# VinAIResearch/Point-Unet

Hardware: AMD Instinct MI355X
Metric: points_per_sec_forward (higher is better)
Workload: dtype f32

## Files before the change

point-unet_amd/csrc/attpool.h:

```cpp
#pragma once

#include "common.h"
#include "rowgemm.h"

namespace ps {

struct Att32Weights {
    const float* w1 = nullptr;
    const float* w2 = nullptr;
    const float* wb1 = nullptr;
    const float* wb2 = nullptr;
    const float* w1b = nullptr;
    const float* w2b = nullptr;
    const float* wb1b = nullptr;
    const float* wb2b = nullptr;
};
void pack_b3(const float* W, int cin, int cout, uint16_t* out);
void pack_b3_locse(const float* W1, int cout, uint16_t* out);
void pack_p32(const float* W, int cin, int cout, float* out);
void pack_p32_locse(const float* W1, int cout, float* out);

struct AttStage {
    const float* xyz = nullptr;
    const int32_t* idx = nullptr;
    const int32_t* order = nullptr;
    const float* fg = nullptr;
    const PackedLinear* lfa1 = nullptr;
    const PackedLinear* lfa2 = nullptr;
    const PackedLinear* wbot = nullptr;
    const PackedLinear* wfull = nullptr;
    int ldf = 0;
    float* agg = nullptr;
    int64_t n_total = 0, n_cloud = 0;
    int d = 0, k = 16;
    const Att32Weights* p32 = nullptr;
};

bool att_pool32_fits(const AttStage& s);
int att_pool32_stage(ps_context* c, const AttStage& s);
bool att_pool32b_fits(const AttStage& s);
int att_pool32b_stage(ps_context* c, const AttStage& s);

int att_pool_stage(ps_context* c, const AttStage& s);
int att_pool16_stage(ps_context* c, const AttStage& s);

}
```

point-unet_amd/csrc/attpool.hip:

```cpp
#include "attpool.h"
#include "mfma_tile.h"

namespace ps {

struct AttArgs {
    const float* xyz;
    const int32_t* idx;
    const int32_t* order;
    const float* fg;
    const float* w1p; const float* b1;
    const float* w2p; const float* b2;
    const float* wbp;
    const float* wfp;
    float* agg;
    int n_total, n_cloud, ldf;
};

struct PointWalk {
    int t, end, stride;
    __device__ __forceinline__ PointWalk(int n_total, int units_per_wg, int unit_in_wg)
    {
        const int per_xcd = (n_total + 7) >> 3;
        const int xcd = blockIdx.x & 7, slot = blockIdx.x >> 3, slots = gridDim.x >> 3;
        t = xcd * per_xcd + slot * units_per_wg + unit_in_wg;
// ... 436 lines not shown
static int dispatch_direct(ps_context* c, int d, const AttArgs& a)
{
    switch (d) {
        case 16: return launch_att_direct<16, STAGE, KN>(c, a);
        case 32: return launch_att_direct<32, STAGE, KN>(c, a);
        default: set_error("att_pool(direct): d_out %d is not a compiled size (16, 32: the weights live in registers)", d); return PS_EINVAL;
    }
}

template <int D, int STAGE, int KN>
static int launch_att(ps_context* c, const AttArgs& a)
{
    constexpr int H = D / 2, PITCH = H + 2;
    constexpr size_t per_wave = (size_t)KN * PITCH * (STAGE == 2 ? 2 : 1) * sizeof(float);
    if (D >= 256 && a.n_total < 16384) {
        constexpr int WAVES = 4;
        const size_t smem = per_wave;
        auto kern = att_kernel<D, STAGE, KN, WAVES, true>;
        if (smem > 48 * 1024) PS_HIP(hipFuncSetAttribute(reinterpret_cast<const void*>(kern), hipFuncAttributeMaxDynamicSharedMemorySize, (int)smem));
        const int blocks = (std::min(a.n_total, 256 * 16) + 7) & ~7;
        hipLaunchKernelGGL(kern, dim3(blocks), dim3(WAVES * 64), smem, c->stream, a);
        PS_HIP(hipGetLastError());
        return PS_OK;
    }
    constexpr int WAVES = per_wave * 4 <= 160 * 1024 ? 4 : (per_wave * 2 <= 160 * 1024 ? 2 : 1);
    static_assert(per_wave * WAVES <= 160 * 1024, "attention tile does not fit the LDS");
    const size_t smem = per_wave * WAVES;
    auto kern = att_kernel<D, STAGE, KN, WAVES, false>;
    if (smem > 48 * 1024) PS_HIP(hipFuncSetAttribute(reinterpret_cast<const void*>(kern), hipFuncAttributeMaxDynamicSharedMemorySize, (int)smem));
    const int blocks = (std::min(ceil_div(a.n_total, WAVES), 256 * 8) + 7) & ~7;
    hipLaunchKernelGGL(kern, dim3(blocks), dim3(WAVES * 64), smem, c->stream, a);
    PS_HIP(hipGetLastError());
    return PS_OK;
}

template <int STAGE, int KN>
static int dispatch_d(ps_context* c, int d, const AttArgs& a)
{
    switch (d) {
        case 16: return launch_att<16, STAGE, KN>(c, a);
        case 32: return launch_att<32, STAGE, KN>(c, a);
        case 64: return launch_att<64, STAGE, KN>(c, a);
        case 128: return launch_att<128, STAGE, KN>(c, a);
        case 256: return launch_att<256, STAGE, KN>(c, a);
        case 512: return launch_att<512, STAGE, KN>(c, a);
        default: set_error("att_pool: d_out %d is not a compiled size (16,32,64,128,256,512)", d); return PS_EINVAL;
    }
}

int att_pool_stage(ps_context* c, const AttStage& s)
{
    if (c->att_bf16x3 && att_pool32b_fits(s)) return att_pool32b_stage(c, s);
    if (att_pool32_fits(s)) return att_pool32_stage(c, s);
    return att_pool16_stage(c, s);
}

int att_pool16_stage(ps_context* c, const AttStage& s)
{
    AttArgs a;
    a.xyz = s.xyz; a.idx = s.idx; a.order = s.order; a.fg = s.fg;
    a.w1p = s.lfa1->wp; a.b1 = s.lfa1->bias;
    a.w2p = s.lfa2 ? s.lfa2->wp : nullptr; a.b2 = s.lfa2 ? s.lfa2->bias : nullptr;
    a.wbp = s.wbot ? s.wbot->wp : nullptr;
    a.wfp = s.wfull ? s.wfull->wp : nullptr;
    a.agg = s.agg;
    a.n_total = (int)s.n_total; a.n_cloud = (int)s.n_cloud;
    a.ldf = s.ldf;
    if (s.n_total <= 0) return PS_OK;
    const int stage = s.lfa2 ? 2 : 1;
    if (s.wfull) {
        PS_CHECK((uint64_t)s.n_total * (uint64_t)std::max(s.d, std::max(s.ldf, 3 * 1)) < (1ull << 32) && (uint64_t)s.n_total * s.k < (1ull << 32),
                 "att_pool: level too large for 32-bit element offsets");
        if (s.k == 16) return stage == 1 ? dispatch_direct<1, 16>(c, s.d, a) : dispatch_direct<2, 16>(c, s.d, a);
        if (s.k == 32) return stage == 1 ? dispatch_direct<1, 32>(c, s.d, a) : dispatch_direct<2, 32>(c, s.d, a);
        set_error("att_pool: k_n %d is not a compiled size (16, 32)", s.k);
        return PS_EINVAL;
    }
    if (s.k == 16) return stage == 1 ? dispatch_d<1, 16>(c, s.d, a) : dispatch_d<2, 16>(c, s.d, a);
    if (s.k == 32) return stage == 1 ? dispatch_d<1, 32>(c, s.d, a) : dispatch_d<2, 32>(c, s.d, a);
    set_error("att_pool: k_n %d is not a compiled size (16, 32)", s.k);
    return PS_EINVAL;
}

}
```

point-unet_amd/csrc/common.h:

```cpp
#pragma once

#include <hip/hip_runtime.h>

#include <cstdarg>
#include <cstdint>
#include <cstdio>
#include <cstring>
#include <map>
#include <string>
#include <vector>

#include "../../include/pointseg.h"
#include "../../include/pointseg_train_ops.h"

namespace ps {

void set_error(const char* fmt, ...);

#define PS_HIP(expr)                                                                                  \
    do {                                                                                              \
        hipError_t _e = (expr);                                                                       \
        if (_e != hipSuccess) {                                                                       \
            ps::set_error("%s failed: %s (%s:%d)", #expr, hipGetErrorString(_e), __FILE__, __LINE__); \
            return PS_EHIP;                                                                           \
// ... 71 lines not shown
int pack_cache_finish_recording(ps_context* c, PackCache& pc);
int pack_cache_replay(ps_context* c, PackCache& pc);
void pack_cache_clear(PackCache& pc);
int pack_batch_ops(ps_context* c, const PackJob* table, int n);
int pack_batch_b3(ps_context* c, const PackJob* table, int n);
}

namespace ps {
struct Tuning {
    double gemm32b_min_flops = 3e8;
    int gemm32b_rw = 0, gemm32b_cw = 0;
    bool gemm32_no_sk8 = false;
    bool att64_gemm = true;
    int att64_occ = 0;
    bool att_no_split = false;
    int64_t wgrad_b3_min_rows = 0;
    int64_t gemm_b3_min_rows = 0;
    int64_t wgrad_wgs = 512;
    bool bn_slice = false;
    bool inv_bucket = true;
    int inv_tile = 4096;
    bool gather_reduce_ordered = true;
    int maxpool_bwd_ordered = 1;
    bool train_act_bf16 = true;
    int train_att_gemm_split = -1;
    bool train_att_gemm = true;
    bool train_att128_fwd_gemm = true;
    bool train_fuse_residual = true;
    bool train_merge_syncbn = true;
    int convbn_max_c = 64;
    int convbn_rect_max = 1 << 30;
    bool wgrad_debug = false;
};
void tuning_from_env(Tuning& t);
}

struct ps_context {
    int device = 0;
    ps::Tuning tune;
    hipStream_t own_stream = nullptr;
    hipStream_t stream = nullptr;
    ps::Arena knn_arena;
    ps::Arena net_arena;
    ps::Arena sample_arena;
    ps::DevBuf stage_in;
    ps::DevBuf stage_out;
    ps::DevBuf red_ws;
    ps::DevBuf wgrad_ws;
    ps::PackCache* pack_cache = nullptr;
    ps::DevBuf ops_ring[4];
    int ops_ring_pos = 0;
    bool att_bf16x3 = true;
    bool regchain_b3 = true;
    bool train_b3 = true;
    bool conv_w_transposed = false;
    bool att_df_accum = false;
    const int32_t* walk_order = nullptr;
    int64_t walk_order_n = 0;
    bool pool_bwd_overwrite = false;
    bool train_bf16 = false;
    bool train_act_bf16 = false;
    bool mid_lds_attr = false;
    size_t chain_lds_attr = 48 * 1024;
    std::map<const void*, size_t> regchain_lds_attr;
    bool deferred = false;
    int32_t* h_flags = nullptr;
    unsigned pending_mask = 0;
    uint64_t builds = 0;
    uint64_t samples = 0;
    uint64_t volume_samples = 0;
    uint64_t flag_serial[8] = {};
    int flag_kind[8] = {};
    int flag_slot = 0;
    int sticky_rc = 0;
    std::string sticky_msg;
    hipEvent_t flag_ev[8] = {};
    std::vector<char> host_ring[8];
    int ring_pos = 0;
    std::vector<char>& ring_next() { ring_pos = (ring_pos + 1) & 7; return host_ring[ring_pos]; }
    int check_deferred();
    int check_flag_slot(int s);
    int defer_status(const void* d_words, size_t bytes, int kind, uint64_t serial);
    struct PinSlot { void* p = nullptr; size_t cap = 0; hipEvent_t ev = nullptr; bool busy = false; };
    PinSlot pin[16];
    int pin_pos = 0;
    int upload_async(void* dst, const void* src, size_t bytes);
    bool timing = false;
    std::string timing_only;
    std::vector<ps::StageTimer> stages;
    std::vector<hipEvent_t> event_pool;
    size_t event_next = 0;
    int cur_stage = -1;
    hipEvent_t cur_start = nullptr;

    hipEvent_t get_event();
    void stage_begin(const char* name);
    void stage_end(int launches);
};

namespace ps {
struct Stage {
    ps_context* c;
    int n;
    bool on = false;
    Stage(ps_context* ctx, const char* name, int launches = 1) : c(ctx), n(launches)
    {
// ... 49 lines not shown
```

point-unet_amd/csrc/context.hip:

```cpp
#include "common.h"
#include "kdtree_build.h"

#include <cstdlib>

namespace ps {

static thread_local char g_err[512] = "";

void set_error(const char* fmt, ...)
{
    va_list ap;
    va_start(ap, fmt);
    vsnprintf(g_err, sizeof g_err, fmt, ap);
    va_end(ap);
}

int DevBuf::reserve(size_t bytes)
{
    if (bytes <= cap) return PS_OK;
    if (p) {
        hipError_t e = hipDeviceSynchronize();
        if (e != hipSuccess) {
            set_error("hipDeviceSynchronize failed: %s", hipGetErrorString(e));
            return PS_EHIP;
// ... 168 lines not shown
    if (num("PS_GEMM32B_MIN_FLOPS", v) && v >= 0) t.gemm32b_min_flops = v;
    if (num("PS_GEMM32B_RW", v) && (v == 1 || v == 2)) t.gemm32b_rw = (int)v;
    if (num("PS_GEMM32B_CW", v) && (v == 1 || v == 2)) t.gemm32b_cw = (int)v;
    t.gemm32_no_sk8 = std::getenv("PS_GEMM32_NO_SK8") != nullptr;
    flag("PS_ATT64_GEMM", t.att64_gemm);
    if (num("PS_ATT64_OCC", v) && (v == 1 || v == 2)) t.att64_occ = (int)v;
    t.att_no_split = std::getenv("PS_ATT_NO_SPLIT") != nullptr;
    clampi("PS_WGRAD_B3_MIN_ROWS", 0, 1ll << 40, t.wgrad_b3_min_rows);
    clampi("PS_GEMM_B3_MIN_ROWS", 0, 1ll << 40, t.gemm_b3_min_rows);
    clampi("PS_WGRAD_WGS", 64, 4096, t.wgrad_wgs);
    flag("PS_BN_SLICE", t.bn_slice);
    flag("PS_INV_BUCKET", t.inv_bucket);
    if (num("PS_INV_TILE", v) && (v == 4096 || v == 6144 || v == 8192)) t.inv_tile = (int)v;
    flag("PS_GATHER_REDUCE_ORDERED", t.gather_reduce_ordered);
    if (num("PS_MAXPOOL_BWD_ORDERED", v)) t.maxpool_bwd_ordered = v != 0;
    flag("PS_TRAIN_ACT_BF16", t.train_act_bf16);
    if (num("PS_TRAIN_ATT_GEMM_SPLIT", v)) t.train_att_gemm_split = v < 0 ? -1 : (v != 0);
    flag("PS_TRAIN_ATT_GEMM", t.train_att_gemm);
    flag("PS_TRAIN_ATT128_FWD_GEMM", t.train_att128_fwd_gemm);
    flag("PS_TRAIN_FUSE_RESIDUAL", t.train_fuse_residual);
    flag("PS_TRAIN_MERGE_SYNCBN", t.train_merge_syncbn);
    if (num("PS_CONVBN_MAX_C", v) && v >= 0 && v <= 4096) t.convbn_max_c = (int)v;
    if (num("PS_CONVBN_RECT_MAX", v) && v >= 0) t.convbn_rect_max = v > (double)(1 << 30) ? 1 << 30 : (int)v;
    t.wgrad_debug = std::getenv("PS_WGRAD_DEBUG") != nullptr;
#else
    (void)t;
#endif
}
}

extern "C" {
const char* ps_version(void) { return "pointseg-hip 0.1 gfx950"; }
int ps_abi_version(void) { return PS_ABI_VERSION; }

int ps_create(int device, ps_context** out)
{
    PS_CHECK(out != nullptr, "ps_create: out is NULL");
    int count = 0;
    PS_HIP(hipGetDeviceCount(&count));
    PS_CHECK(device >= 0 && device < count, "ps_create: device %d out of range (%d devices)", device, count);
    PS_HIP(hipSetDevice(device));
    ps_context* c = new ps_context();
    c->device = device;
    hipError_t e = hipStreamCreateWithFlags(&c->own_stream, hipStreamNonBlocking);
    if (e != hipSuccess) {
        delete c;
        ps::set_error("hipStreamCreate failed: %s", hipGetErrorString(e));
        return PS_EHIP;
    }
    c->stream = c->own_stream;
    ps::tuning_from_env(c->tune);
#ifdef PS_TUNING_ENV
    if (const char* v = std::getenv("PS_REGCHAIN_B3")) c->regchain_b3 = std::atof(v) != 0;
#endif
    *out = c;
    return PS_OK;
}

int ps_destroy(ps_context* c)
{
    if (!c) return PS_OK;
    (void)hipSetDevice(c->device);
    (void)hipStreamSynchronize(c->stream);
    c->knn_arena.buf.release();
    c->net_arena.buf.release();
    c->sample_arena.buf.release();
    c->stage_in.release();
    c->stage_out.release();
    c->red_ws.release();
    c->wgrad_ws.release();
    for (auto& b : c->ops_ring) b.release();
    if (c->h_flags) (void)hipHostFree(c->h_flags);
    for (auto& e : c->flag_ev)
        if (e) (void)hipEventDestroy(e);
    for (auto& s : c->pin) {
        if (s.p) (void)hipHostFree(s.p);
        if (s.ev) (void)hipEventDestroy(s.ev);
    }
    for (hipEvent_t e : c->event_pool) (void)hipEventDestroy(e);
    if (c->own_stream) (void)hipStreamDestroy(c->own_stream);
    delete c;
    return PS_OK;
}

int ps_set_stream(ps_context* c, void* hip_stream)
{
    PS_CHECK(c != nullptr, "ps_set_stream: ctx is NULL");
    c->stream = static_cast<hipStream_t>(hip_stream);
    return PS_OK;
}

int ps_synchronize(ps_context* c)
{
    PS_CHECK(c != nullptr, "ps_synchronize: ctx is NULL");
    PS_HIP(hipStreamSynchronize(c->stream));
    return c->check_deferred();
}

int ps_set_train_gemm_bf16(ps_context* c, int on)
{
    PS_CHECK(c != nullptr, "ps_set_train_gemm_bf16: ctx is NULL");
    c->train_bf16 = on != 0;
    return PS_OK;
}

int ps_set_train_act_bf16(ps_context* c, int on)
// ... 75 lines not shown
```

point-unet_amd/csrc/debug_hooks.h:

```cpp
#ifndef POINTSEG_DEBUG_H
#define POINTSEG_DEBUG_H
#include "../../include/pointseg.h"
#ifdef __cplusplus
extern "C" {
#endif
int ps_debug_knn_host(const float* support, const float* queries, int64_t B, int64_t n_support,
                      int64_t n_queries, int64_t K, int32_t* out_idx);
int ps_debug_kdtree_host(const float* support, int64_t n, int32_t* vind, int32_t* nodes, float* pts,
                         int32_t* root_depth, float* bbox);
int ps_debug_kdtree_device(ps_context* ctx, const float* support, int64_t n, int32_t* vind, int32_t* nodes,
                           float* pts, int32_t* root_depth, float* bbox);
#define PS_DEBUG_KDTREE_STATS 22
int ps_debug_kdtree_device_set(ps_context* ctx, const float* support, const int32_t* n, int64_t T, const int32_t* want_copy, int32_t* vind,
                               int32_t* nodes, float* pts, int32_t* fat, int32_t* root_depth, float* bbox, float* copy, int32_t* stats);
int ps_debug_pack_weights(const float* W, int cin, int cout, int ntb, float* out);
int ps_debug_pack_b3(const float* W, int cin, int cout, uint16_t* out);
int ps_debug_gemm32(ps_context* ctx, int split_bf16, const float* x1, int ld1, int c1, const int32_t* g1, const float* x2, int ld2, int c2,
                    const int32_t* g2, int gm, int gn, const float* W, const float* bias, int64_t R, int cout, int leaky, float* y, int ldy);
int ps_debug_gemm32_plan(ps_context* ctx, int split_bf16, int64_t R, int cin, int cout, int* out4);

typedef struct ps_debug_chain_layer {
    const float* W;
    const float* bias;
    int cin, cout, leaky;
    float* y;
    int ldy;
    const float* extra;
    int ld_extra, c_extra;
    const int32_t* extra_gather;
} ps_debug_chain_layer;
typedef struct ps_debug_chain_desc {
    int n_layers;
    ps_debug_chain_layer layer[4];
    const float* x1; const int32_t* g1; int ld1, c1, g1m, g1n;
    const float* x2; const int32_t* g2; int ld2, c2, g2m, g2n;
    int64_t R;
} ps_debug_chain_desc;
int ps_debug_chain(ps_context* ctx, const ps_debug_chain_desc* d, int form);
int ps_debug_chain_plan(const ps_debug_chain_desc* d, int* out4);
int ps_debug_set_regchain_b3(ps_context* ctx, int on);
int ps_debug_att_stage(ps_randla* net, int level, int stage, int form, const float* xyz, const int32_t* idx, const int32_t* order, const float* fg,
                       int64_t n_total, int64_t n_cloud, float* agg);

int ps_debug_set_tuning(ps_context* ctx, const char* field, double value);
int ps_debug_get_tuning(ps_context* ctx, const char* field, double* value);
int ps_debug_tuning_fields(char* buf, int cap);
int ps_debug_volume_sample_args_size(void);

int64_t ps_debug_scan_words(int64_t n);
int64_t ps_debug_sort_words(int64_t n);
int ps_debug_scan_launches(int64_t n);
int ps_debug_sort_launches(int64_t n, int bits);
int ps_debug_scan_u32(ps_context* ctx, const uint32_t* in, uint32_t* out, int64_t n, uint32_t* work);
int ps_debug_sort_pairs(ps_context* ctx, int key_bytes, void* k0, void* k1, uint32_t* v0, uint32_t* v1, int64_t n, int bits, uint32_t* work,
                        int* which_out);
int ps_debug_reduce_partials(ps_context* ctx, int form, const void* part, int n_part, int nv, int n0, void* out0, void* out1);

#ifdef __cplusplus
}
#endif
#endif
```

point-unet_amd/csrc/debug_hooks.hip:

```cpp
#include "common.h"

#include <cstring>
#include <vector>
#include "kdtree_build.h"
#include "kdtree_host.h"
#include "rowgemm.h"
#include "attpool.h"
#include "debug_hooks.h"
#include "randla_net.h"
#include "reduce_partials.h"
#include "sortscan.h"

using namespace ps;

extern "C" int ps_debug_volume_sample_args_size(void) { return (int)sizeof(ps_volume_sample_args); }

extern "C" int ps_debug_pack_weights(const float* W, int cin, int cout, int ntb, float* out)
{
    PS_CHECK(W && out && (ntb == 1 || ntb == 2 || ntb == 4), "ps_debug_pack_weights: bad argument");
    pack_weights(W, cin, cout, ntb, out);
    return PS_OK;
}

extern "C" int ps_debug_pack_b3(const float* W, int cin, int cout, uint16_t* out)
// ... 149 lines not shown
    float* dev = nullptr;
    PS_HIP(hipMalloc(reinterpret_cast<void**>(&dev), total * sizeof(float)));
    int rc = PS_OK;
    if (hipMemcpyAsync(dev, host.data(), host.size() * sizeof(float), hipMemcpyHostToDevice, c->stream) != hipSuccess) {
        set_error("ps_debug_chain: upload failed");
        rc = PS_EHIP;
    }
    for (int i = 0; i < b.n; ++i) {
        b.L[i].wp = dev + wp_off[i];
        b.L[i].bias = dev + b_off[i];
        b.L[i].wq = wq_off[i] ? dev + wq_off[i] : nullptr;
    }
    if (rc == PS_OK) {
        if (form == 0) {
            ChainCache cache;
            if (rowchain_fits(b.steps, b.n, b.s1, b.s2)) rc = rowchain(c, b.steps, b.n, b.s1, b.s2, d->R, &cache);
            else { set_error("ps_debug_chain: the chain fits neither chain kernel (channels above %d, mismatched, or a gathered extra)", kChainMaxC); rc = PS_EINVAL; }
            (void)hipStreamSynchronize(c->stream);
            cache.clear();
        } else if (form == 1) {
            if (regchain_fits(b.steps, b.n, b.s1, b.s2)) rc = regchain(c, b.steps, b.n, b.s1, b.s2, d->R, nullptr);
            else { set_error("ps_debug_chain: not one of regchain's compiled chain shapes"); rc = PS_EINVAL; }
        } else if (form == 2) {
            if (rowchain_lds_plan(b.steps, b.n, b.s1, b.s2, d->R).form == 2) rc = rowchain_lds(c, b.steps, b.n, b.s1, b.s2, d->R);
            else { set_error("ps_debug_chain: the chain does not fit the LDS-staged kernel (channels above %d, mismatched, or a gathered extra)", kChainMaxC); rc = PS_EINVAL; }
        } else {
            RowSrc in1 = b.s1, in2 = b.s2;
            for (int i = 0; i < b.n && rc == PS_OK; ++i) {
                const ChainStep& st = b.steps[i];
                if (i > 0) {
                    in2 = RowSrc();
                    if (st.extra.x) in2 = st.extra;
                }
                float* out = st.y ? st.y : dev + tmp_off[i];
                const int ldo = st.y ? st.ldy : b.L[i].cout;
                rc = rowgemm(c, b.L[i], in1, in2, d->R, out, ldo);
                in1 = RowSrc();
                in1.x = out; in1.ld = ldo; in1.c = b.L[i].cout;
            }
        }
    }
    (void)hipStreamSynchronize(c->stream);
    (void)hipFree(dev);
    return rc;
}

extern "C" int ps_debug_set_regchain_b3(ps_context* c, int on)
{
    PS_CHECK(c && (on == 0 || on == 1), "ps_debug_set_regchain_b3: bad argument");
    c->regchain_b3 = on != 0;
    return PS_OK;
}

extern "C" int ps_debug_att_stage(ps_randla* net, int level, int stage, int form, const float* xyz, const int32_t* idx, const int32_t* order,
                                  const float* fg, int64_t n_total, int64_t n_cloud, float* agg)
{
    PS_CHECK(net && xyz && idx && fg && agg, "ps_debug_att_stage: NULL argument");
    PS_CHECK(net->have_weights, "ps_debug_att_stage: weights not set");
    PS_CHECK(level >= 0 && level < net->cfg.num_layers && (stage == 1 || stage == 2) && form >= 0 && form <= 3, "ps_debug_att_stage: bad level / stage / form");
    PS_CHECK(n_total >= 0 && n_cloud >= 1 && n_total % n_cloud == 0, "ps_debug_att_stage: n_total must be a whole number of clouds");
    ps_context* c = net->ctx;
    PS_HIP(hipSetDevice(c->device));
    const EncLevel& e = net->enc[level];
    const int d = e.d, h = d / 2;
    const bool use_g = d >= 64;
    AttStage s;
    s.xyz = xyz; s.idx = idx; s.order = order; s.fg = fg; s.lfa1 = &e.lfa1; s.agg = agg;
    s.n_total = n_total; s.n_cloud = n_cloud; s.d = d; s.k = net->cfg.k_n; s.ldf = use_g ? h + d : h;
    s.p32 = e.has_p32 ? &e.p32 : nullptr;
    s.lfa2 = stage == 2 ? &e.lfa2 : nullptr;
    s.wbot = use_g ? (stage == 1 ? &e.bot1 : &e.bot2) : nullptr;
    s.wfull = use_g ? nullptr : (stage == 1 ? &e.full1 : &e.full2);
    int rc = PS_EINVAL;
    if (form == 0) rc = att_pool_stage(c, s);
    else if (form == 1 && att_pool32b_fits(s)) rc = att_pool32b_stage(c, s);
    else if (form == 2 && att_pool32_fits(s)) rc = att_pool32_stage(c, s);
    else if (form == 3) rc = att_pool16_stage(c, s);
    else set_error("ps_debug_att_stage: the level (d = %d, %lld rows) does not fit the 32x32 form %d", d, (long long)n_total, form);
    (void)hipStreamSynchronize(c->stream);
    return rc;
}

static bool is_bool(double v) { return v == 0 || v == 1; }
static bool is_int_in(double v, double lo, double hi) { return v >= lo && v <= hi && v == (double)(int64_t)v; }

#define PS_TUNING_FIELDS(X)                                                \
    X(gemm32b_min_flops, v >= 0 && v <= 1e300)                             \
    X(gemm32b_rw, v == 0 || v == 1 || v == 2)                              \
    X(gemm32b_cw, v == 0 || v == 1 || v == 2)                              \
    X(gemm32_no_sk8, is_bool(v))                                           \
    X(att64_gemm, is_bool(v))                                              \
    X(att64_occ, v == 0 || v == 1 || v == 2)                               \
    X(att_no_split, is_bool(v))                                            \
    X(wgrad_b3_min_rows, is_int_in(v, 0, (double)(1ll << 40)))             \
    X(gemm_b3_min_rows, is_int_in(v, 0, (double)(1ll << 40)))              \
    X(wgrad_wgs, is_int_in(v, 64, 4096))                                   \
    X(bn_slice, is_bool(v))                                                \
    X(inv_bucket, is_bool(v))                                              \
    X(inv_tile, v == 4096 || v == 6144 || v == 8192)                       \
    X(gather_reduce_ordered, is_bool(v))                                   \
    X(maxpool_bwd_ordered, is_bool(v))                                     \
    X(train_act_bf16, is_bool(v))                                          \
    X(train_att_gemm_split, v == -1 || v == 0 || v == 1)                   \
    X(train_att_gemm, is_bool(v))                                          \
    X(train_att128_fwd_gemm, is_bool(v))                                   \
    X(train_fuse_residual, is_bool(v))                                     \
    X(train_merge_syncbn, is_bool(v))                                      \
    X(convbn_max_c, is_int_in(v, 0, 4096))                                 \
    X(convbn_rect_max, is_int_in(v, 0, (double)(1 << 30)))                 \
    X(wgrad_debug, is_bool(v))

extern "C" int ps_debug_set_tuning(ps_context* c, const char* field, double v)
{
    PS_CHECK(c && field, "ps_debug_set_tuning: NULL argument");
#define PS_SET(f, ok)                                                                                 \
    if (std::strcmp(field, #f) == 0) {                                                                \
        PS_CHECK(ok, "ps_debug_set_tuning: %g is not a value %s is compiled for", v, #f);             \
        c->tune.f = static_cast<decltype(c->tune.f)>(v);                                              \
        return PS_OK;                                                                                 \
    }
    PS_TUNING_FIELDS(PS_SET)
#undef PS_SET
    PS_CHECK(false, "ps_debug_set_tuning: no knob named '%s'", field);
}

extern "C" int ps_debug_get_tuning(ps_context* c, const char* field, double* out)
{
    PS_CHECK(c && field && out, "ps_debug_get_tuning: NULL argument");
#define PS_GET(f, ok)                               \
    if (std::strcmp(field, #f) == 0) {              \
        *out = static_cast<double>(c->tune.f);      \
        return PS_OK;                               \
    }
    PS_TUNING_FIELDS(PS_GET)
// ... 188 lines not shown
```

point-unet_amd/csrc/randla.hip:

```cpp
#include "attpool.h"
#include "common.h"
#include "randla_net.h"
#include "rowgemm.h"

#include <memory>

namespace ps {

template <int KN>
__global__ __launch_bounds__(256) void pool_max_kernel(const float* __restrict__ feat, const int32_t* __restrict__ idx, const int32_t* __restrict__ order,
                                                       float* __restrict__ out, int rows_out, int m_cloud, int n_cloud, int K, int c4 ,
                                                       unsigned char* __restrict__ ties )
{
    const int per_xcd = (rows_out + 7) >> 3;
    const int xcd = blockIdx.x & 7;
    const size_t lim = (size_t)min(rows_out, (xcd + 1) * per_xcd) * c4;
    for (size_t t = (size_t)xcd * per_xcd * c4 + (size_t)(blockIdx.x >> 3) * 256 + threadIdx.x; t < lim; t += (size_t)(gridDim.x >> 3) * 256) {
        const int r = (int)(t / c4), q = (int)(t - (size_t)r * c4);
        const int row = order ? (r / m_cloud) * m_cloud + order[r] : r;
        const int base = (row / m_cloud) * n_cloud;
        const int32_t* ix = idx + (size_t)row * K;
        const float4* f4 = reinterpret_cast<const float4*>(feat);
        float4 m;
        if constexpr (KN > 0) {
// ... 193 lines not shown
        return host.data() + off;
    };
    size_t si = 0;
    auto W = [&](size_t i) { return blob + net->specs[i].w_off; };
    auto Bv = [&](size_t i) { return blob + net->specs[i].b_off; };
    const ps_randla_config& cfg = net->cfg;
    emit(net->fc0, W(si), Bv(si), cfg.in_channels, 8, 1);
    ++si;
    net->enc.assign(cfg.num_layers, EncLevel());
    int d_in = 8;
    std::vector<float> tmp;
    for (int i = 0; i < cfg.num_layers; ++i) {
        EncLevel& e = net->enc[i];
        const int d = cfg.d_out[i], h = d / 2;
        e.d = d; e.d_in = d_in;
        e.has_p32 = d >= 64;
        if (e.has_p32) {
            pack_p32_locse(W(si + 1), h, emit_raw(&e.p32.w1, (size_t)(h / 32) * 5 * 64));
            auto scaled = [&](const float* src, size_t count) {
                tmp.resize(count);
                for (size_t t = 0; t < count; ++t) tmp[t] = (float)((double)src[t] * 1.4426950408889634);
                return tmp.data();
            };
            pack_p32(scaled(W(si + 2) + (size_t)h * d, (size_t)h * d), h, d, emit_raw(&e.p32.wb1, (size_t)h * d));
            pack_p32(W(si + 4), h, h, emit_raw(&e.p32.w2, (size_t)h * h));
            pack_p32(scaled(W(si + 5) + (size_t)h * d, (size_t)h * d), h, d, emit_raw(&e.p32.wb2, (size_t)h * d));
            if (d == 64 || d == 128 || d == 256 || d == 512) {
                pack_b3_locse(W(si + 1), h, reinterpret_cast<uint16_t*>(emit_raw(&e.p32.w1b, (size_t)(h / 32) * 3 * 64 * 4)));
                pack_b3(scaled(W(si + 2) + (size_t)h * d, (size_t)h * d), h, d, reinterpret_cast<uint16_t*>(emit_raw(&e.p32.wb1b, (size_t)h * d * 3 / 2)));
                pack_b3(W(si + 4), h, h, reinterpret_cast<uint16_t*>(emit_raw(&e.p32.w2b, (size_t)h * h * 3 / 2)));
                pack_b3(scaled(W(si + 5) + (size_t)h * d, (size_t)h * d), h, d, reinterpret_cast<uint16_t*>(emit_raw(&e.p32.wb2b, (size_t)h * d * 3 / 2)));
            }
        }
        emit(e.mlp1, W(si), Bv(si), d_in, h, 1); ++si;
        emit(e.lfa1, W(si), Bv(si), 10, h, 1); ++si;
        emit(e.top1, W(si), nullptr, h, d, 0);
        emit(e.bot1, W(si) + (size_t)h * d, nullptr, h, d, 0);
        {
            std::vector<float> sc((size_t)d * d);
            for (size_t t = 0; t < sc.size(); ++t) sc[t] = (float)((double)W(si)[t] * 1.4426950408889634);
            emit(e.full1, sc.data(), nullptr, d, d, 0);
        }
        ++si;
        emit(e.att1mlp, W(si), Bv(si), d, h, 1); ++si;
        emit(e.lfa2, W(si), Bv(si), h, h, 1); ++si;
        emit(e.top2, W(si), nullptr, h, d, 0);
        emit(e.bot2, W(si) + (size_t)h * d, nullptr, h, d, 0);
        {
            std::vector<float> sc((size_t)d * d);
            for (size_t t = 0; t < sc.size(); ++t) sc[t] = (float)((double)W(si)[t] * 1.4426950408889634);
            emit(e.full2, sc.data(), nullptr, d, d, 0);
        }
        ++si;
        emit(e.att2mlp, W(si), Bv(si), d, d, 1); ++si;
        tmp.assign((size_t)(d + d_in) * 2 * d + 2 * d, 0.f);
        std::memcpy(tmp.data(), W(si), sizeof(float) * (size_t)d * 2 * d);
        std::memcpy(tmp.data() + (size_t)d * 2 * d, W(si + 1), sizeof(float) * (size_t)d_in * 2 * d);
        float* bsum = tmp.data() + (size_t)(d + d_in) * 2 * d;
        for (int k = 0; k < 2 * d; ++k) bsum[k] = Bv(si)[k] + Bv(si + 1)[k];
        emit(e.mlp2sc, tmp.data(), bsum, d + d_in, 2 * d, 1);
        si += 2;
        d_in = 2 * d;
    }
    emit(net->decoder0, W(si), Bv(si), d_in, d_in, 1); ++si;
    net->dec.assign(cfg.num_layers, PackedLinear());
    for (int j = 0; j < cfg.num_layers; ++j) {
        emit(net->dec[j], W(si), Bv(si), net->specs[si].cin, net->specs[si].cout, 1);
        ++si;
    }
    emit(net->fc1, W(si), Bv(si), net->specs[si].cin, 64, 1); ++si;
    emit(net->fc2, W(si), Bv(si), 64, 32, 1); ++si;
    emit(net->fc, W(si), Bv(si), 32, cfg.num_classes, 0); ++si;

    PS_TRY(net->wbuf.reserve(host.size() * sizeof(float)));
    PS_HIP(hipMemcpyAsync(net->wbuf.p, host.data(), host.size() * sizeof(float), hipMemcpyHostToDevice, c->stream));
    PS_HIP(hipStreamSynchronize(c->stream));
    for (auto& p : pend) {
        p.L->wp = net->wbuf.as<float>() + p.wp_off;
        p.L->bias = net->wbuf.as<float>() + p.b_off;
        p.L->wq = p.wq_off ? net->wbuf.as<float>() + p.wq_off : nullptr;
        p.L->w32 = p.w32_off ? net->wbuf.as<float>() + p.w32_off : nullptr;
        p.L->w32b = p.w32b_off ? net->wbuf.as<float>() + p.w32b_off : nullptr;
    }
    for (auto& p : pend_raw) *p.dst = net->wbuf.as<float>() + p.off;
    net->have_weights = true;
    return PS_OK;
}

extern "C" int ps_randla_forward(ps_randla* net, const ps_pyramid* pyr, const float* features, float* logits)
{
    PS_CHECK(net && pyr && features && logits, "ps_randla_forward: NULL argument");
    if (!net->have_weights) {
        set_error("ps_randla_forward: weights not set");
        return PS_ESTATE;
    }
    ps_context* c = net->ctx;
    const ps_randla_config& cfg = net->cfg;
    const int L = cfg.num_layers;
    PS_CHECK(pyr->num_layers == L && pyr->K == cfg.k_n, "ps_randla_forward: pyramid (layers %d, K %d) does not match the network (%d, %d)",
             pyr->num_layers, pyr->K, L, cfg.k_n);
    PS_HIP(hipSetDevice(c->device));
    const int64_t B = pyr->B;
    const int64_t* n = pyr->n;

    Arena& A = c->net_arena;
    float *fc0 = nullptr, *fg = nullptr, *agg = nullptr, *tmp = nullptr, *dec0 = nullptr, *h1 = nullptr, *h2 = nullptr;
// ... 12 lines not shown
        fg = A.take<float>(fg_max);
        agg = A.take<float>(agg_max);
        tmp = A.take<float>(agg_max);
        dec0 = A.take<float>((size_t)B * n[L] * 2 * cfg.d_out[L - 1]);
        for (int j = 0; j < L; ++j) decb[j] = A.take<float>((size_t)B * n[L - 1 - j] * net->dec[j].cout);
        h1 = A.take<float>((size_t)B * n[0] * 64);
        h2 = A.take<float>((size_t)B * n[0] * 32);
        if (pass == 0) PS_TRY(A.buf.reserve(A.off));
    }
    net->taps.clear();
    auto tap = [&](int which, const float* p, int64_t count) { net->taps.push_back({which, p, count}); };

    const RowSrc none;
    auto src = [](const float* x, int ld, int ch) {
        RowSrc s;
        s.x = x; s.ld = ld; s.c = ch;
        return s;
    };

    auto step = [](const PackedLinear& Lr, float* y, int ldy) {
        ChainStep st;
        st.L = &Lr; st.y = y; st.ldy = ldy;
        return st;
    };
    const int d0 = net->enc[0].d, ldf0 = d0 >= 64 ? d0 / 2 + d0 : d0 / 2;
    bool mlp1_0_done = false;
    {
        ChainStep ch[2] = {step(net->fc0, fc0, 8), step(net->enc[0].mlp1, fg, ldf0)};
        const RowSrc in = src(features, cfg.in_channels, cfg.in_channels);
        if (rowchain_fits(ch, 2, in, none)) {
            Stage st(c, "fc0", 1);
            PS_TRY(rowchain(c, ch, 2, in, none, B * n[0], &net->chains));
            mlp1_0_done = true;
        } else {
            Stage st(c, "fc0", 1);
            PS_TRY(rowgemm(c, net->fc0, in, none, B * n[0], fc0, 8));
        }
    }
    tap(0, fc0, B * n[0] * 8);

    const float* X = fc0;
    int d_in = 8;
    for (int i = 0; i < L; ++i) {
        const EncLevel& e = net->enc[i];
        const int d = e.d, h = d / 2;
        const int64_t R = B * n[i];
        const bool use_g = d >= 64;
        const int ldf = use_g ? h + d : h;
        char nm[48];
        AttStage s;
        s.xyz = pyr->xyz[i]; s.idx = pyr->neigh_idx[i]; s.order = pyr->order[i]; s.fg = fg; s.lfa1 = &e.lfa1; s.agg = agg;
        s.n_total = R; s.n_cloud = n[i]; s.d = d; s.k = cfg.k_n; s.ldf = ldf;
        s.p32 = e.has_p32 ? &e.p32 : nullptr;
        auto feature_rows = [&](const PackedLinear& mlp, const PackedLinear& top, const RowSrc& in) -> int {
            ChainStep ch[2] = {step(mlp, fg, ldf), step(top, fg + h, ldf)};
            const int nsteps = use_g ? 2 : 1;
            if (nsteps == 2 && rowchain_fits(ch, 2, in, none)) return rowchain(c, ch, 2, in, none, R, &net->chains);
            if (nsteps == 1 && regchain_fits(ch, 1, in, none)) return rowchain(c, ch, 1, in, none, R, &net->chains);
            PS_TRY(rowgemm(c, mlp, in, none, R, fg, ldf));
            if (use_g) PS_TRY(rowgemm(c, top, src(fg, ldf, h), none, R, fg + h, ldf));
            return PS_OK;
        };
        if (i == 0 && mlp1_0_done) {
            if (use_g) {
                std::snprintf(nm, sizeof nm, "enc%d_dense", i);
                Stage st(c, nm, 1);
                PS_TRY(rowgemm(c, e.top1, src(fg, ldf, h), none, R, fg + h, ldf));
            }
        } else {
            std::snprintf(nm, sizeof nm, "enc%d_dense", i);
            Stage st(c, nm, 1);
            PS_TRY(feature_rows(e.mlp1, e.top1, src(X, d_in, d_in)));
        }
        {
            std::snprintf(nm, sizeof nm, "enc%d_att1", i);
            Stage st(c, nm, 1);
            s.lfa2 = nullptr; s.wbot = use_g ? &e.bot1 : nullptr; s.wfull = use_g ? nullptr : &e.full1;
            PS_TRY(att_pool_stage(c, s));
        }
        {
            std::snprintf(nm, sizeof nm, "enc%d_dense", i);
            Stage st(c, nm, 1);
            PS_TRY(feature_rows(e.att1mlp, e.top2, src(agg, d, d)));
        }
        {
            std::snprintf(nm, sizeof nm, "enc%d_att2", i);
            Stage st(c, nm, 1);
            s.lfa2 = &e.lfa2; s.wbot = use_g ? &e.bot2 : nullptr; s.wfull = use_g ? nullptr : &e.full2;
            PS_TRY(att_pool_stage(c, s));
        }
        {
            std::snprintf(nm, sizeof nm, "enc%d_dense", i);
            Stage st(c, nm, 1);
            ChainStep ch[2] = {step(e.att2mlp, nullptr, 0), step(e.mlp2sc, encb[i], 2 * d)};
            ch[1].extra = src(X, d_in, d_in);
            const RowSrc in = src(agg, d, d);
            if (rowchain_fits(ch, 2, in, none)) {
                PS_TRY(rowchain(c, ch, 2, in, none, R, &net->chains));
            } else {
                PS_TRY(rowgemm(c, e.att2mlp, in, none, R, tmp, d));
                PS_TRY(rowgemm(c, e.mlp2sc, src(tmp, d, d), src(X, d_in, d_in), R, encb[i], 2 * d));
            }
        }
        {
            std::snprintf(nm, sizeof nm, "enc%d_pool", i);
            Stage st(c, nm, 1);
            PS_TRY(pool_max(c, encb[i], pyr->sub_idx[i], i + 1 < L ? pyr->order[i + 1] : nullptr, poolb[i], B, n[i], n[i + 1], cfg.k_n, 2 * d));
        }
        tap(10 + i, encb[i], R * 2 * d);
        tap(20 + i, poolb[i], B * n[i + 1] * 2 * d);
        X = poolb[i];
        d_in = 2 * d;
    }

    {
        Stage st(c, "decoder_0", 1);
        PS_TRY(rowgemm(c, net->decoder0, src(X, d_in, d_in), none, B * n[L], dec0, d_in));
    }
    tap(30, dec0, B * n[L] * d_in);

    const float* up = dec0;
    int up_c = d_in;
    for (int j = 0; j < L; ++j) {
        const int lvl = L - 1 - j;
        const float* skip = lvl == 0 ? encb[0] : poolb[lvl - 1];
        const int skip_c = net->dec[j].cout;
        RowSrc s2 = src(up, up_c, up_c);
        s2.gather = pyr->interp_idx[lvl];
        s2.gm = (int)n[lvl];
        s2.gn = (int)n[lvl + 1];
        char nm[48];
        std::snprintf(nm, sizeof nm, "dec%d", j);
        if (j == L - 1) {
            ChainStep ch[4] = {step(net->dec[j], net->keep_taps ? decb[j] : nullptr, skip_c), step(net->fc1, nullptr, 0), step(net->fc2, nullptr, 0),
                               step(net->fc, logits, cfg.num_classes)};
            const RowSrc s1 = src(skip, skip_c, skip_c);
            if (rowchain_fits(ch, 4, s1, s2)) {
                Stage st(c, "head", 1);
                PS_TRY(rowchain(c, ch, 4, s1, s2, B * n[lvl], &net->chains));
                if (net->keep_taps) tap(40 + j, decb[j], B * n[lvl] * skip_c);
                return PS_OK;
// ... 38 lines not shown
```

point-unet_amd/csrc/randla_net.h:

```cpp
#pragma once

#include <vector>

#include "attpool.h"
#include "common.h"
#include "rowgemm.h"

namespace ps {

struct LayerSpec {
    int cin, cout, leaky;
    size_t w_off, b_off;
};

struct EncLevel {
    PackedLinear mlp1, top1, lfa1, bot1, full1, att1mlp, lfa2, top2, bot2, full2, att2mlp, mlp2sc;
    Att32Weights p32;
    bool has_p32 = false;
    int d_in, d;
};

}

struct ps_randla {
    ps_context* ctx = nullptr;
    ps_randla_config cfg;
    std::vector<ps::LayerSpec> specs;
    int64_t blob_floats = 0;
    bool have_weights = false;
    ps::DevBuf wbuf;
    ps::ChainCache chains;
    ps::PackedLinear fc0, decoder0, fc1, fc2, fc;
    std::vector<ps::EncLevel> enc;
    std::vector<ps::PackedLinear> dec;
    struct Tap { int which; const float* p; int64_t count; };
    std::vector<Tap> taps;
    bool keep_taps = false;
};
```

Baseline: 192.0 million.

## Add lane-per-neighbor attentive pooling kernel for d=16 levels with scalar-loaded weight image

```diff
diff --git a/point-unet_amd/csrc/attpool.h b/point-unet_amd/csrc/attpool.h
--- a/point-unet_amd/csrc/attpool.h
+++ b/point-unet_amd/csrc/attpool.h
@@ -34,14 +34,23 @@
     int64_t n_total = 0, n_cloud = 0;
     int d = 0, k = 16;
     const Att32Weights* p32 = nullptr;
+    const float* lane = nullptr;
 };
+
+constexpr int kLaneB1 = 0, kLaneW1 = 8, kLaneB2 = 88, kLaneW2 = 96, kLaneWfc = 160, kLaneImageFloats = 416;
+void pack_lane_image(const float* W1, const float* b1, const float* W2, const float* b2, const float* wfc_scaled, float* out);
 
 bool att_pool32_fits(const AttStage& s);
 int att_pool32_stage(ps_context* c, const AttStage& s);
 bool att_pool32b_fits(const AttStage& s);
 int att_pool32b_stage(ps_context* c, const AttStage& s);
 
+bool att_lane_fits(const ps_context* c, const AttStage& s);
+int att_lane_stage(ps_context* c, const AttStage& s);
+int att_lane_pass_points();
+
 int att_pool_stage(ps_context* c, const AttStage& s);
+int att_pool_form(const ps_context* c, const AttStage& s);
 int att_pool16_stage(ps_context* c, const AttStage& s);
 
 }
diff --git a/point-unet_amd/csrc/attpool.hip b/point-unet_amd/csrc/attpool.hip
--- a/point-unet_amd/csrc/attpool.hip
+++ b/point-unet_amd/csrc/attpool.hip
@@ -512,7 +512,15 @@
 {
     if (c->att_bf16x3 && att_pool32b_fits(s)) return att_pool32b_stage(c, s);
     if (att_pool32_fits(s)) return att_pool32_stage(c, s);
+    if (att_lane_fits(c, s)) return att_lane_stage(c, s);
     return att_pool16_stage(c, s);
+}
+
+int att_pool_form(const ps_context* c, const AttStage& s)
+{
+    if (c->att_bf16x3 && att_pool32b_fits(s)) return 1;
+    if (att_pool32_fits(s)) return 2;
+    return att_lane_fits(c, s) ? 4 : 3;
 }
 
 int att_pool16_stage(ps_context* c, const AttStage& s)
diff --git a/point-unet_amd/csrc/attpool_lane.hip b/point-unet_amd/csrc/attpool_lane.hip
--- /dev/null
+++ b/point-unet_amd/csrc/attpool_lane.hip
@@ -0,0 +1,198 @@
+#include "attpool.h"
+#include "mfma_tile.h"
+
+namespace ps {
+
+void pack_lane_image(const float* W1, const float* b1, const float* W2, const float* b2, const float* wfc_scaled, float* out)
+{
+    std::memcpy(out + kLaneB1, b1, sizeof(float) * 8);
+    std::memcpy(out + kLaneW1, W1, sizeof(float) * 80);
+    if (b2) std::memcpy(out + kLaneB2, b2, sizeof(float) * 8);
+    else std::memset(out + kLaneB2, 0, sizeof(float) * 8);
+    if (W2) std::memcpy(out + kLaneW2, W2, sizeof(float) * 64);
+    else std::memset(out + kLaneW2, 0, sizeof(float) * 64);
+    std::memcpy(out + kLaneWfc, wfc_scaled, sizeof(float) * 256);
+}
+
+namespace {
+
+struct AttLaneArgs {
+    const float* xyz;
+    const int32_t* idx;
+    const int32_t* order;
+    const float* f;
+    const float* w;
+    float* agg;
+    int n_total, n_cloud, ldf;
+};
+
+constexpr int kLaneWaves = 4;
+constexpr int kLanePts = 4;
+constexpr int kLaneMaxBlocks = 256 * 8;
+constexpr int kLanePitch = 17;
+
+static_assert(kLaneB1 == 0 && kLaneW1 == 8 && kLaneB2 == 88 && kLaneW2 == 96 && kLaneWfc == 160 && kLaneImageFloats == 13 * 32, "att_lane_kernel: image layout");
+
+using cfloat = const float __attribute__((address_space(4)));
+using cfloat2 = const f32x2 __attribute__((address_space(4)));
+
+__device__ __forceinline__ f32x2 fma2(float x, f32x2 w, f32x2 acc) { return __builtin_elementwise_fma(f32x2{x, x}, w, acc); }
+__device__ __forceinline__ f32x2 leaky2(f32x2 v) { return f32x2{leaky02(v.x), leaky02(v.y)}; }
+
+template <int STAGE>
+__global__ __launch_bounds__(kLaneWaves * 64) void att_lane_kernel(AttLaneArgs a)
+{
+    __shared__ float smem[kLaneWaves * 64 * kLanePitch];
+    const int wave = __builtin_amdgcn_readfirstlane(threadIdx.x >> 6), lane = threadIdx.x & 63;
+    const int pi = lane >> 4, k = lane & 15;
+    float* T = smem + wave * (64 * kLanePitch);
+    float* t_row = T + lane * kLanePitch;
+    const float* t_col = T + (pi * 16) * kLanePitch + k;
+    cfloat* wimg = (cfloat*)(uintptr_t)a.w;
+
+    const bool one_cloud = a.n_total == a.n_cloud;
+    const int per_xcd = ((((a.n_total + 7) >> 3) + kLanePts - 1) / kLanePts) * kLanePts;
+    const int w_end = min(a.n_total, (int)((blockIdx.x & 7) + 1) * per_xcd), w_slots = gridDim.x >> 3;
+    for (int t = (int)(blockIdx.x & 7) * per_xcd + ((int)(blockIdx.x >> 3) * kLaneWaves + wave) * kLanePts; t < w_end; t += w_slots * kLaneWaves * kLanePts) {
+        const int ti = min(t + pi, w_end - 1);
+        unsigned p, base;
+        if (one_cloud) {
+            p = a.order ? (unsigned)a.order[ti] : (unsigned)ti;
+            base = 0u;
+        } else {
+            base = ((unsigned)ti / (unsigned)a.n_cloud) * (unsigned)a.n_cloud;
+            p = a.order ? base + (unsigned)a.order[ti] : (unsigned)ti;
+        }
+        const float* cp = a.xyz + 3u * p;
+        const float cx = cp[0], cy = cp[1], cz = cp[2];
+        const unsigned nb = base + (unsigned)a.idx[p * 16u + (unsigned)k];
+        const float* np = a.xyz + 3u * nb;
+        const float nx = np[0], ny = np[1], nz = np[2];
+        const float4* fr = reinterpret_cast<const float4*>(a.f + nb * (unsigned)a.ldf);
+        const float4 fa = fr[0], fb = fr[1];
+        const float rx = cx - nx, ry = cy - ny, rz = cz - nz;
+        const float dis = __builtin_amdgcn_sqrtf(rx * rx + ry * ry + rz * rz);
+        const float enc[10] = {dis, rx, ry, rz, cx, cy, cz, nx, ny, nz};
+
+        f32x2 w[2][16];
+        auto fetch = [&](int c, f32x2 (&dst)[16], auto& after) {
+            cfloat* wp = wimg;
+            asm volatile("" : "+s"(wp), "+v"(after));
+            cfloat2* w2 = reinterpret_cast<cfloat2*>(wp) + c * 16;
+#pragma unroll
+            for (int j = 0; j < 16; ++j) dst[j] = w2[j];
+        };
+        auto mac4 = [](float xv, const f32x2* wr, f32x2 (&acc)[4]) {
+#pragma unroll
+            for (int j = 0; j < 4; ++j) acc[j] = fma2(xv, wr[j], acc[j]);
+        };
+        int tie = ti;
+        fetch(0, w[0], tie);
+        fetch(1, w[1], tie);
+        f32x2 fx[4], g2[4];
+#pragma unroll
+        for (int j = 0; j < 4; ++j) fx[j] = w[0][j];
+#pragma unroll
+        for (int q = 0; q < 3; ++q) mac4(enc[q], &w[0][4 + 4 * q], fx);
+        fetch(2, w[0], fx[0]);
+#pragma unroll
+        for (int q = 3; q < 7; ++q) mac4(enc[q], &w[1][4 * (q - 3)], fx);
+        fetch(STAGE == 2 ? 3 : 5, w[1], fx[0]);
+#pragma unroll
+        for (int q = 7; q < 10; ++q) mac4(enc[q], &w[0][4 * (q - 7)], fx);
+#pragma unroll
+        for (int j = 0; j < 4; ++j) {
+            g2[j] = w[0][12 + j];
+            fx[j] = leaky2(fx[j]);
+        }
+        if constexpr (STAGE == 2) {
+            fetch(4, w[0], g2[0]);
+#pragma unroll
+            for (int q = 0; q < 4; ++q) mac4(q & 1 ? fx[q >> 1].y : fx[q >> 1].x, &w[1][4 * q], g2);
+            fetch(5, w[1], g2[0]);
+#pragma unroll
+            for (int q = 4; q < 8; ++q) mac4(q & 1 ? fx[q >> 1].y : fx[q >> 1].x, &w[0][4 * (q - 4)], g2);
+#pragma unroll
+            for (int j = 0; j < 4; ++j) fx[j] = leaky2(g2[j]);
+        }
+        const float x[16] = {fa.x, fa.y, fa.z, fa.w, fb.x, fb.y, fb.z, fb.w, fx[0].x, fx[0].y, fx[1].x, fx[1].y, fx[2].x, fx[2].y, fx[3].x, fx[3].y};
+        f32x2 s[8];
+#pragma unroll
+        for (int j = 0; j < 8; ++j) s[j] = f32x2{0.f, 0.f};
+#pragma unroll
+        for (int i = 0; i < 8; ++i) {
+            if (i < 7) fetch(6 + i, w[i & 1], s[0]);
+            const f32x2* wr = w[(i + 1) & 1];
+#pragma unroll
+            for (int j = 0; j < 8; ++j) s[j] = fma2(x[2 * i], wr[j], s[j]);
+#pragma unroll
+            for (int j = 0; j < 8; ++j) s[j] = fma2(x[2 * i + 1], wr[8 + j], s[j]);
+        }
+#pragma unroll
+        for (int j = 0; j < 8; ++j) {
+            t_row[2 * j] = s[j].x;
+            t_row[2 * j + 1] = s[j].y;
+        }
+        wave_lds_sync();
+        float sc[16];
+#pragma unroll
+        for (int r = 0; r < 16; ++r) sc[r] = t_col[r * kLanePitch];
+        wave_lds_sync();
+#pragma unroll
+        for (int q = 0; q < 16; ++q) t_row[q] = x[q];
+        wave_lds_sync();
+        float v[16];
+#pragma unroll
+        for (int r = 0; r < 16; ++r) v[r] = t_col[r * kLanePitch];
+        wave_lds_sync();
+        float m = sc[0];
+#pragma unroll
+        for (int r = 1; r < 16; ++r) m = fmaxf(m, sc[r]);
+        float ss[4], num[4];
+#pragma unroll
+        for (int g = 0; g < 4; ++g) {
+            ss[g] = 0.f;
+            num[g] = 0.f;
+#pragma unroll
+            for (int r = 4 * g; r < 4 * g + 4; ++r) {
+                const float e = __builtin_amdgcn_exp2f(sc[r] - m);
+                ss[g] += e;
+                num[g] = __builtin_fmaf(e, v[r], num[g]);
+            }
+        }
+        const float ssum = (ss[0] + ss[1]) + (ss[2] + ss[3]);
+        const float nsum = (num[0] + num[1]) + (num[2] + num[3]);
+        if (t + pi < w_end) a.agg[p * 16u + (unsigned)k] = nsum * __builtin_amdgcn_rcpf(ssum);
+    }
+}
+
+}
+
+int att_lane_pass_points() { return kLaneMaxBlocks * kLaneWaves * kLanePts; }
+
+bool att_lane_fits(const ps_context* c, const AttStage& s)
+{
+    return c->att_lane && s.wfull && s.lane && s.d == 16 && s.k == 16 && s.ldf >= 8 && s.ldf % 4 == 0 &&
+           (uint64_t)s.n_total * (uint64_t)std::max(s.d, std::max(s.ldf, 3)) < (1ull << 32);
+}
+
+int att_lane_stage(ps_context* c, const AttStage& s)
+{
+    if (!(s.wfull && s.lane && s.d == 16 && s.k == 16)) {
+        set_error("att_pool(lane): d_out %d, k_n %d -- the lane kernel is compiled for d_out 16, k_n 16 and the direct formulation only", s.d, s.k);
+        return PS_EINVAL;
+    }
+    PS_CHECK((uint64_t)s.n_total * (uint64_t)std::max(s.d, std::max(s.ldf, 3)) < (1ull << 32), "att_pool(lane): level too large for 32-bit element offsets");
+    PS_CHECK(s.ldf % 4 == 0 && s.ldf >= 8, "att_pool(lane): feature rows need a stride of whole float4s");
+    if (s.n_total <= 0) return PS_OK;
+    AttLaneArgs a;
+    a.xyz = s.xyz; a.idx = s.idx; a.order = s.order; a.f = s.fg; a.w = s.lane; a.agg = s.agg;
+    a.n_total = (int)s.n_total; a.n_cloud = (int)s.n_cloud; a.ldf = s.ldf;
+    const int blocks = (std::min(ceil_div(a.n_total, kLaneWaves * kLanePts), kLaneMaxBlocks) + 7) & ~7;
+    if (s.lfa2) hipLaunchKernelGGL(att_lane_kernel<2>, dim3(blocks), dim3(kLaneWaves * 64), 0, c->stream, a);
+    else hipLaunchKernelGGL(att_lane_kernel<1>, dim3(blocks), dim3(kLaneWaves * 64), 0, c->stream, a);
+    PS_HIP(hipGetLastError());
+    return PS_OK;
+}
+
+}
diff --git a/point-unet_amd/csrc/common.h b/point-unet_amd/csrc/common.h
--- a/point-unet_amd/csrc/common.h
+++ b/point-unet_amd/csrc/common.h
@@ -147,6 +147,7 @@
     int ops_ring_pos = 0;
     bool att_bf16x3 = true;
     bool regchain_b3 = true;
+    bool att_lane = true;
     bool train_b3 = true;
     bool conv_w_transposed = false;
     bool att_df_accum = false;
diff --git a/point-unet_amd/csrc/context.hip b/point-unet_amd/csrc/context.hip
--- a/point-unet_amd/csrc/context.hip
+++ b/point-unet_amd/csrc/context.hip
@@ -244,6 +244,7 @@
     ps::tuning_from_env(c->tune);
 #ifdef PS_TUNING_ENV
     if (const char* v = std::getenv("PS_REGCHAIN_B3")) c->regchain_b3 = std::atof(v) != 0;
+    if (const char* v = std::getenv("PS_ATT_LANE")) c->att_lane = std::atof(v) != 0;
 #endif
     *out = c;
     return PS_OK;
diff --git a/point-unet_amd/csrc/debug_hooks.h b/point-unet_amd/csrc/debug_hooks.h
--- a/point-unet_amd/csrc/debug_hooks.h
+++ b/point-unet_amd/csrc/debug_hooks.h
@@ -39,8 +39,11 @@
 int ps_debug_chain(ps_context* ctx, const ps_debug_chain_desc* d, int form);
 int ps_debug_chain_plan(const ps_debug_chain_desc* d, int* out4);
 int ps_debug_set_regchain_b3(ps_context* ctx, int on);
+int ps_debug_set_att_lane(ps_context* ctx, int on);
 int ps_debug_att_stage(ps_randla* net, int level, int stage, int form, const float* xyz, const int32_t* idx, const int32_t* order, const float* fg,
                        int64_t n_total, int64_t n_cloud, float* agg);
+int ps_debug_att_form(ps_randla* net, int level, int stage, int k, int64_t n_total);
+int ps_debug_att_lane_pass_points(void);
 
 int ps_debug_set_tuning(ps_context* ctx, const char* field, double value);
 int ps_debug_get_tuning(ps_context* ctx, const char* field, double* value);
diff --git a/point-unet_amd/csrc/debug_hooks.hip b/point-unet_amd/csrc/debug_hooks.hip
--- a/point-unet_amd/csrc/debug_hooks.hip
+++ b/point-unet_amd/csrc/debug_hooks.hip
@@ -225,12 +225,19 @@
     return PS_OK;
 }
 
+extern "C" int ps_debug_set_att_lane(ps_context* c, int on)
+{
+    PS_CHECK(c && (on == 0 || on == 1), "ps_debug_set_att_lane: bad argument");
+    c->att_lane = on != 0;
+    return PS_OK;
+}
+
 extern "C" int ps_debug_att_stage(ps_randla* net, int level, int stage, int form, const float* xyz, const int32_t* idx, const int32_t* order,
                                   const float* fg, int64_t n_total, int64_t n_cloud, float* agg)
 {
     PS_CHECK(net && xyz && idx && fg && agg, "ps_debug_att_stage: NULL argument");
     PS_CHECK(net->have_weights, "ps_debug_att_stage: weights not set");
-    PS_CHECK(level >= 0 && level < net->cfg.num_layers && (stage == 1 || stage == 2) && form >= 0 && form <= 3, "ps_debug_att_stage: bad level / stage / form");
+    PS_CHECK(level >= 0 && level < net->cfg.num_layers && (stage == 1 || stage == 2) && form >= 0 && form <= 4, "ps_debug_att_stage: bad level / stage / form");
     PS_CHECK(n_total >= 0 && n_cloud >= 1 && n_total % n_cloud == 0, "ps_debug_att_stage: n_total must be a whole number of clouds");
     ps_context* c = net->ctx;
     PS_HIP(hipSetDevice(c->device));
@@ -244,8 +251,10 @@
     s.lfa2 = stage == 2 ? &e.lfa2 : nullptr;
     s.wbot = use_g ? (stage == 1 ? &e.bot1 : &e.bot2) : nullptr;
     s.wfull = use_g ? nullptr : (stage == 1 ? &e.full1 : &e.full2);
+    s.lane = stage == 1 ? e.lane1 : e.lane2;
     int rc = PS_EINVAL;
-    if (form == 0) rc = att_pool_stage(c, s);
+    if (form == 4) rc = att_lane_stage(c, s);
+    else if (form == 0) rc = att_pool_stage(c, s);
     else if (form == 1 && att_pool32b_fits(s)) rc = att_pool32b_stage(c, s);
     else if (form == 2 && att_pool32_fits(s)) rc = att_pool32_stage(c, s);
     else if (form == 3) rc = att_pool16_stage(c, s);
@@ -253,6 +262,27 @@
     (void)hipStreamSynchronize(c->stream);
     return rc;
 }
+
+extern "C" int ps_debug_att_form(ps_randla* net, int level, int stage, int k, int64_t n_total)
+{
+    if (!net || !net->have_weights || level < 0 || level >= net->cfg.num_layers || (stage != 1 && stage != 2) || k < 1 || n_total < 0) {
+        set_error("ps_debug_att_form: bad argument");
+        return -1;
+    }
+    const EncLevel& e = net->enc[level];
+    const int d = e.d, h = d / 2;
+    const bool use_g = d >= 64;
+    AttStage s;
+    s.lfa1 = &e.lfa1; s.lfa2 = stage == 2 ? &e.lfa2 : nullptr;
+    s.wbot = use_g ? (stage == 1 ? &e.bot1 : &e.bot2) : nullptr;
+    s.wfull = use_g ? nullptr : (stage == 1 ? &e.full1 : &e.full2);
+    s.lane = stage == 1 ? e.lane1 : e.lane2;
+    s.p32 = e.has_p32 ? &e.p32 : nullptr;
+    s.n_total = n_total; s.n_cloud = n_total; s.d = d; s.k = k; s.ldf = use_g ? h + d : h;
+    return att_pool_form(net->ctx, s);
+}
+
+extern "C" int ps_debug_att_lane_pass_points(void) { return att_lane_pass_points(); }
 
 static bool is_bool(double v) { return v == 0 || v == 1; }
 static bool is_int_in(double v, double lo, double hi) { return v >= lo && v <= hi && v == (double)(int64_t)v; }
diff --git a/point-unet_amd/csrc/randla.hip b/point-unet_amd/csrc/randla.hip
--- a/point-unet_amd/csrc/randla.hip
+++ b/point-unet_amd/csrc/randla.hip
@@ -269,6 +269,17 @@
             emit(e.full2, sc.data(), nullptr, d, d, 0);
         }
         ++si;
+        e.lane1 = e.lane2 = nullptr;
+        if (d == 16) {
+            auto scaled16 = [&](const float* src) {
+                tmp.resize(256);
+                for (size_t t = 0; t < 256; ++t) tmp[t] = (float)((double)src[t] * 1.4426950408889634);
+                return tmp.data();
+            };
+            const size_t lfa1_i = si - 5, fc1_i = si - 4, lfa2_i = si - 2, fc2_i = si - 1;
+            pack_lane_image(W(lfa1_i), Bv(lfa1_i), nullptr, nullptr, scaled16(W(fc1_i)), emit_raw(&e.lane1, kLaneImageFloats));
+            pack_lane_image(W(lfa1_i), Bv(lfa1_i), W(lfa2_i), Bv(lfa2_i), scaled16(W(fc2_i)), emit_raw(&e.lane2, kLaneImageFloats));
+        }
         emit(e.att2mlp, W(si), Bv(si), d, d, 1); ++si;
         tmp.assign((size_t)(d + d_in) * 2 * d + 2 * d, 0.f);
         std::memcpy(tmp.data(), W(si), sizeof(float) * (size_t)d * 2 * d);
@@ -387,6 +398,7 @@
         s.xyz = pyr->xyz[i]; s.idx = pyr->neigh_idx[i]; s.order = pyr->order[i]; s.fg = fg; s.lfa1 = &e.lfa1; s.agg = agg;
         s.n_total = R; s.n_cloud = n[i]; s.d = d; s.k = cfg.k_n; s.ldf = ldf;
         s.p32 = e.has_p32 ? &e.p32 : nullptr;
+        s.lane = e.lane1;
         auto feature_rows = [&](const PackedLinear& mlp, const PackedLinear& top, const RowSrc& in) -> int {
             ChainStep ch[2] = {step(mlp, fg, ldf), step(top, fg + h, ldf)};
             const int nsteps = use_g ? 2 : 1;
@@ -422,6 +434,7 @@
             std::snprintf(nm, sizeof nm, "enc%d_att2", i);
             Stage st(c, nm, 1);
             s.lfa2 = &e.lfa2; s.wbot = use_g ? &e.bot2 : nullptr; s.wfull = use_g ? nullptr : &e.full2;
+            s.lane = e.lane2;
             PS_TRY(att_pool_stage(c, s));
         }
         {
diff --git a/point-unet_amd/csrc/randla_net.h b/point-unet_amd/csrc/randla_net.h
--- a/point-unet_amd/csrc/randla_net.h
+++ b/point-unet_amd/csrc/randla_net.h
@@ -17,6 +17,7 @@
     PackedLinear mlp1, top1, lfa1, bot1, full1, att1mlp, lfa2, top2, bot2, full2, att2mlp, mlp2sc;
     Att32Weights p32;
     bool has_p32 = false;
+    const float *lane1 = nullptr, *lane2 = nullptr;
     int d_in, d;
 };
 
```

Result: faster. 198.5 million (median of 6 runs) (+3.4%).
